# FlagArihant2000/sfm-mvs

Hardware: AMD Instinct MI355X
Metric: descriptor-pair distances/sec (BF-KNN k=2 + Lowe ratio) (higher is better)
Workload: dtype f32 results (bit-identical to the direct-form f32 reference); filter arithmetic on MFMA: i8 MFMA on the descriptors QUANTISED to 8 bits (one grid per pair; the certificate uses the measured residua...; 1 GPU; BASELINE configs[1]: 10k x 10k uniform[0,1) float32 128-D descriptors, BF-KNN k=2 + Lowe ratio 0.70; a step = one launch set = a batch of 8 distinct pairs of that shape per GPU (8e8 distances; 8 distinct pairs per launch set, 2 sets of images rotating over the steps); nq=10000, nt=10000, dim=128

## Files before the change

include/sfm_hip.h:

```cpp
#ifndef SFM_HIP_H
#define SFM_HIP_H

#include <stddef.h>
#include <stdint.h>

#ifdef __cplusplus
extern "C" {
#endif

#define SFM_ABI_VERSION 3

#define SFM_OK             0
#define SFM_ERR_ARG       -1
#define SFM_ERR_WORKSPACE -2
#define SFM_ERR_DEVICE    -3

int         sfm_abi_version(void);
const char* sfm_last_error(void);
const char* sfm_build_id(void);

#define SFM_KNN_FILTER_AUTO      0
#define SFM_KNN_FILTER_F32       1
#define SFM_KNN_FILTER_SPLIT     2
#define SFM_KNN_FILTER_LDS       3
// ... 142 lines not shown
int sfm_host_p3p(const double* K_host, const double* Xw_host, const double* uv_host, double* R_host, double* t_host,
                 int32_t* ok_host);
int sfm_host_five_point(const double* x1n_host, const double* x2n_host, double* E_host, int32_t* count_host);
int sfm_host_decompose_essential(const double* E_host, double* R1_host, double* R2_host, double* t_host);
int sfm_host_pnp_dlt_init(const double* K_host, const double* X_host, const double* uv_host, int64_t n,
                          double* rvec_host, double* tvec_host, int32_t* status_host);
int sfm_host_rodrigues(const double* src_host, int src_is_matrix, double* dst_host, double* jac_host);

int sfm_bgr2gray_u8(const uint8_t* bgr_dev, int64_t w, int64_t h, int64_t stride_bytes, uint8_t* gray_dev, void* stream);
int sfm_pyrdown_u8(const uint8_t* src_dev, int64_t w, int64_t h, int channels, uint8_t* dst_dev, void* stream);
size_t sfm_sift_ws_bytes(int64_t w, int64_t h, int n_octave_layers, int64_t max_keypoints);
int sfm_sift_detect_and_compute(const uint8_t* gray_dev, int64_t w, int64_t h, int64_t stride_bytes,
                                int n_octave_layers, double contrast_threshold, double edge_threshold,
                                double sigma, int64_t max_keypoints, float* keypoints_dev,
                                float* descriptors_dev, int32_t* count_dev, void* ws, size_t ws_bytes,
                                void* stream);

int sfm_mvs_plane_sweep(const uint8_t* ref_dev, const uint8_t* const* src_dev, const float* mv_host, int nsrc, int64_t w, int64_t h,
                        const float* invd_dev, int ndepth, int radius, int topk, float var_min, float cost_max,
                        float* depth_dev, float* cost_dev, int32_t* plane_dev, float* volume_dev, void* stream);
int sfm_mvs_consistency(const float* depth_dev, const float* const* nbr_depth_dev, const int32_t* nbr_index_host,
                        const float* ab_host, int nview, int ref_index, const float* bc_host, int64_t w, int64_t h, float tau,
                        int min_consistent, int unique, uint8_t* mask_dev, float* xyz_dev, void* stream);

int sfm_mvs_cost_shift(const float* volume_dev, int64_t w, int64_t h, int ndepth, int shift, uint16_t* q_dev, void* stream);
int sfm_mvs_cost_aggregate(const uint16_t* q_dev, int64_t w, int64_t h, int ndepth, int p1, int p2, int ndir, uint16_t* s_dev,
                           void* stream);
int sfm_mvs_cost_depth(const uint16_t* s_dev, const uint16_t* q_dev, const float* invd_dev, int64_t w, int64_t h, int ndepth, int gate,
                       float* depth_dev, float* cost_dev, int32_t* plane_dev, void* stream);

int sfm_tsdf_integrate(const float* depth_dev, const uint8_t* mask_dev, const uint8_t* bgr_dev, const float* P_dev, int nview, int64_t w,
                       int64_t h, const float* origin_host, float voxel, int64_t nx, int64_t ny, int64_t nz, float trunc, float* S_dev,
                       float* W_dev, float* CWc_dev, void* stream);
size_t sfm_mesh_count_ws_bytes(int64_t nx, int64_t ny, int64_t nz);
int sfm_mesh_count(const float* S_dev, const float* W_dev, int64_t nx, int64_t ny, int64_t nz, float w_min, int32_t* counts_dev,
                   void* ws_dev, size_t ws_bytes, void* stream);
size_t sfm_mesh_extract_ws_bytes(int64_t nx, int64_t ny, int64_t nz);
int sfm_mesh_extract(const float* S_dev, const float* W_dev, const float* CWc_dev, const float* origin_host, float voxel, int64_t nx,
                     int64_t ny, int64_t nz, float w_min, int64_t max_vertices, int64_t max_faces, float* vertices_dev, float* colors_dev,
                     int32_t* faces_dev, void* ws_dev, size_t ws_bytes, void* stream);

size_t sfm_mesh_components_ws_bytes(int64_t nv, int64_t nf);
int sfm_mesh_components(const int32_t* faces_dev, int64_t nv, int64_t nf, int rounds, int resume, int32_t* labels_dev, int32_t* status_dev,
                        void* ws_dev, size_t ws_bytes, void* stream);
size_t sfm_mesh_clean_ws_bytes(int64_t nv, int64_t nf);
int sfm_mesh_clean(const float* vertices_dev, const float* colors_dev, const int32_t* faces_dev, int64_t nv, int64_t nf,
                   const int32_t* labels_dev, int64_t min_faces, int largest_only, float* out_vertices_dev, float* out_colors_dev,
                   int32_t* out_faces_dev, int32_t* counts_dev, void* ws_dev, size_t ws_bytes, void* stream);

int sfm_profile_enable(int on);
int sfm_debug_set_trace(void* dev_buf);
int sfm_debug_knn_split_delay(int workgroup, int microseconds);
int sfm_debug_knn_prep_general(int on);
int sfm_profile_read(int slot, double* total_ms_host, int64_t* launches_host);
int64_t sfm_host_sync_count(void);
int sfm_pnp_profile_read(double* out10_host, int reset);
int64_t sfm_host_poll_count(void);
int sfm_debug_pnp_sweep_server(int on);

#ifdef __cplusplus
}
#endif
#endif
```

sfm_mvs_amd/_lib.py:

```python
import ctypes
import os

import torch

_HERE = os.path.dirname(os.path.abspath(__file__))
LIB_PATH = os.environ.get("SFM_HIP_LIB") or os.path.join(_HERE, "lib", "libsfmhip.so")

ABI_VERSION = 3


class SfmHipError(RuntimeError):
    """A libsfmhip.so entry point returned a negative status."""


_c = ctypes
_i64, _i32, _int, _f32, _f64, _sz, _vp = (_c.c_int64, _c.c_int32, _c.c_int, _c.c_float, _c.c_double,
                                          _c.c_size_t, _c.c_void_p)

SIGNATURES = {
    "sfm_abi_version": (_int, []),
    "sfm_last_error": (_c.c_char_p, []),
    "sfm_build_id": (_c.c_char_p, []),
    "sfm_knn2_l2_f32_ws_bytes": (_sz, [_i64, _i64, _int, _int]),
    "sfm_knn2_l2_f32": (_int, [_vp, _i64, _i64, _vp, _i64, _i64, _int, _int, _vp, _vp, _vp, _vp, _sz, _vp]),
# ... 23 lines not shown
    "sfm_ba_schur_solve": (_int, [_vp, _i64, _vp, _vp, _i64, _i64, _vp, _vp, _vp, _vp, _f64, _int, _f64, _int, _vp, _vp,
                                  _c.POINTER(_i32), _c.POINTER(_i32), _vp, _sz, _vp]),
    "sfm_ba_schur_indexed_ws_bytes": (_sz, [_i64]),
    "sfm_ba_schur_indexed": (_int, [_vp, _i64, _vp, _vp, _i64, _i64, _vp, _vp, _i64, _int, _vp, _vp, _vp, _sz, _vp]),
    "sfm_block_inverse": (_int, [_vp, _i64, _int, _vp, _vp]),
    "sfm_block_inverse_checked": (_int, [_vp, _i64, _int, _vp, _vp, _vp]),
    "sfm_block_matvec": (_int, [_vp, _vp, _i64, _int, _vp, _vp]),
    "sfm_norm_l2_ws_bytes": (_sz, []),
    "sfm_norm_l2": (_int, [_vp, _vp, _i64, _int, _vp, _vp, _sz, _vp]),
    "sfm_host_epnp": (_int, [_vp, _vp, _vp, _int, _vp, _vp]),
    "sfm_selftest_mfma_accumulation": (_int, [_int, _int, _vp, _vp, _sz, _vp]),
    "sfm_knn_mfma_selftest_result": (_int, [_c.POINTER(_f64), _c.POINTER(_f32)]),
    "sfm_host_p3p": (_int, [_vp, _vp, _vp, _vp, _vp, _vp]),
    "sfm_host_five_point": (_int, [_vp, _vp, _vp, _vp]),
    "sfm_host_decompose_essential": (_int, [_vp, _vp, _vp, _vp]),
    "sfm_host_pnp_dlt_init": (_int, [_vp, _vp, _vp, _i64, _vp, _vp, _vp]),
    "sfm_host_rodrigues": (_int, [_vp, _int, _vp, _vp]),
    "sfm_project_points_f64": (_int, [_vp, _vp, _vp, _vp, _i64, _vp, _vp]),
    "sfm_find_essential_mat_ws_bytes": (_sz, [_i64]),
    "sfm_find_essential_mat": (_int, [_vp, _vp, _i64, _vp, _f64, _f64, _int, _vp, _vp, _vp, _vp, _sz, _vp]),
    "sfm_recover_pose_ws_bytes": (_sz, [_i64]),
    "sfm_recover_pose": (_int, [_vp, _vp, _vp, _i64, _vp, _f64, _int, _vp, _vp, _vp, _vp, _vp, _sz, _vp]),
    "sfm_solve_pnp_ransac_ws_bytes": (_sz, [_i64]),
    "sfm_solve_pnp_ransac": (_int, [_vp, _vp, _i64, _vp, _int, _f32, _f64, _vp, _vp, _vp, _vp, _vp, _sz, _vp]),
    "sfm_bgr2gray_u8": (_int, [_vp, _i64, _i64, _i64, _vp, _vp]),
    "sfm_pyrdown_u8": (_int, [_vp, _i64, _i64, _int, _vp, _vp]),
    "sfm_sift_ws_bytes": (_sz, [_i64, _i64, _int, _i64]),
    "sfm_sift_detect_and_compute": (_int, [_vp, _i64, _i64, _i64, _int, _f64, _f64, _f64, _i64, _vp, _vp, _vp, _vp, _sz, _vp]),
    "sfm_score_essential": (_int, [_vp, _int, _vp, _vp, _i64, _f32, _vp, _vp, _vp]),
    "sfm_recover_pose_score": (_int, [_vp, _int, _vp, _vp, _i64, _f64, _int, _vp, _vp, _vp]),
    "sfm_score_pnp": (_int, [_vp, _int, _vp, _vp, _vp, _i64, _f32, _vp, _vp, _vp]),
    "sfm_mvs_plane_sweep": (_int, [_vp, _vp, _vp, _int, _i64, _i64, _vp, _int, _int, _int, _f32, _f32, _vp, _vp, _vp, _vp, _vp]),
    "sfm_mvs_consistency": (_int, [_vp, _vp, _vp, _vp, _int, _int, _vp, _i64, _i64, _f32, _int, _int, _vp, _vp, _vp]),
    "sfm_mvs_cost_shift": (_int, [_vp, _i64, _i64, _int, _int, _vp, _vp]),
    "sfm_mvs_cost_aggregate": (_int, [_vp, _i64, _i64, _int, _int, _int, _int, _vp, _vp]),
    "sfm_mvs_cost_depth": (_int, [_vp, _vp, _vp, _i64, _i64, _int, _int, _vp, _vp, _vp, _vp]),
    "sfm_tsdf_integrate": (_int, [_vp, _vp, _vp, _vp, _int, _i64, _i64, _vp, _f32, _i64, _i64, _i64, _f32, _vp, _vp, _vp, _vp]),
    "sfm_mesh_count_ws_bytes": (_sz, [_i64, _i64, _i64]),
    "sfm_mesh_count": (_int, [_vp, _vp, _i64, _i64, _i64, _f32, _vp, _vp, _sz, _vp]),
    "sfm_mesh_extract_ws_bytes": (_sz, [_i64, _i64, _i64]),
    "sfm_mesh_extract": (_int, [_vp, _vp, _vp, _vp, _f32, _i64, _i64, _i64, _f32, _i64, _i64, _vp, _vp, _vp, _vp, _sz, _vp]),
    "sfm_mesh_components_ws_bytes": (_sz, [_i64, _i64]),
    "sfm_mesh_components": (_int, [_vp, _i64, _i64, _int, _int, _vp, _vp, _vp, _sz, _vp]),
    "sfm_mesh_clean_ws_bytes": (_sz, [_i64, _i64]),
    "sfm_mesh_clean": (_int, [_vp, _vp, _vp, _i64, _i64, _vp, _i64, _int, _vp, _vp, _vp, _vp, _vp, _sz, _vp]),
    "sfm_profile_enable": (_int, [_int]),
    "sfm_host_sync_count": (_i64, []),
    "sfm_pnp_profile_read": (_int, [_c.POINTER(_f64), _int]),
    "sfm_host_poll_count": (_i64, []),
    "sfm_debug_pnp_sweep_server": (_int, [_int]),
    "sfm_debug_set_trace": (_int, [_vp]),
    "sfm_debug_knn_split_delay": (_int, [_int, _int]),
    "sfm_debug_knn_prep_general": (_int, [_int]),
    "sfm_profile_read": (_int, [_int, _c.POINTER(_f64), _c.POINTER(_i64)]),
}

_lib = None


def lib():
    global _lib
    if _lib is not None:
        return _lib
    if not os.path.exists(LIB_PATH):
        raise ImportError(
            f"{LIB_PATH} is missing: the HIP extension has not been built. "
            "Run `python -c 'import __graft_entry__ as g; g.build()'` (or `make -C sfm_mvs_amd/csrc`). "
            "There is no CPU fallback for the hot path.")
    handle = ctypes.CDLL(LIB_PATH)
    handle.sfm_abi_version.restype = _int
    handle.sfm_abi_version.argtypes = []
    got = handle.sfm_abi_version()
    if got != ABI_VERSION:
        raise ImportError(f"{LIB_PATH}: ABI {got} != binding ABI {ABI_VERSION}; rebuild (python -c 'import __graft_entry__ as g; g.build()')")
    for name, (res, args) in SIGNATURES.items():
        try:
            fn = getattr(handle, name)
        except AttributeError as e:
            raise ImportError(f"{LIB_PATH} (ABI {got}) does not export {name}: header / library mismatch; rebuild") from e
        fn.restype = res
        fn.argtypes = args
    _lib = handle
    return _lib


def build_id():
    return lib().sfm_build_id().decode()


def code_hashes_of_binary():
    return dict(tok.split(":", 1) for tok in build_id().split() if ":" in tok)


def knn_code_hash_of_binary():
    return build_id().split(":", 1)[1].split()[0]


def check(rc, what):
    if rc != 0:
        msg = lib().sfm_last_error()
        raise SfmHipError(f"{what} failed (status {rc}): {msg.decode() if msg else '?'}")


def require_cuda(*tensors):
    for t in tensors:
        if t is not None and not t.is_cuda:
# ... 38 lines not shown
```

sfm_mvs_amd/csrc/knn.hip:

```cpp
#include "common.h"
#include <cfloat>
#include <climits>
#include <cstdlib>
#include <type_traits>
#include <algorithm>
#include <mutex>
#include <vector>

namespace {

typedef float f32x16 __attribute__((ext_vector_type(16)));
typedef float f32x4 __attribute__((ext_vector_type(4)));
typedef float f32x3 __attribute__((ext_vector_type(3), aligned(4)));
typedef int i32x3 __attribute__((ext_vector_type(3), aligned(4)));

constexpr int kDim = 128;
constexpr int kTileT = 32;


constexpr int kResidentWaves = 4096;
constexpr int kMaxSlots = 258;
constexpr float kInf = __builtin_huge_valf();
constexpr int kSubTilesHost = 64;
constexpr int kI8SubTilesHost = 128;
// ... 425 lines not shown
                k1 = m1;
                k0 = lo;
                (void)hi;
            }
            if (!(ABL & 2)) __syncthreads();
        }

        if (qok) {
            flush_keys(k0, k1, k2, sub_t0, h, cand_s + obase + 6 * sub, cand_i + obase + 6 * sub);
            for (int e = sub + 1; e < nsub; ++e)
#pragma unroll
                for (int r = 0; r < 3; ++r) {
                    cand_s[obase + 6 * e + r] = kInf;
                    cand_i[obase + 6 * e + r] = -1;
                }
        }
        u += t_end - t_begin;
    }
    if (trace && threadIdx.x == 0) trace[4 * blockIdx.x + 1] = wall_clock64();
}

typedef __bf16 bf16x8 __attribute__((ext_vector_type(8)));
typedef _Float16 f16x8 __attribute__((ext_vector_type(8)));
typedef unsigned u32x4 __attribute__((ext_vector_type(4)));
typedef _Float16 f16x2 __attribute__((ext_vector_type(2)));
typedef float f32x2 __attribute__((ext_vector_type(2)));

__device__ __forceinline__ float dot8_f16(const uint4& a, const uint4& b, float c) {
    c = __builtin_amdgcn_fdot2(__builtin_bit_cast(f16x2, a.x), __builtin_bit_cast(f16x2, b.x), c, false);
    c = __builtin_amdgcn_fdot2(__builtin_bit_cast(f16x2, a.y), __builtin_bit_cast(f16x2, b.y), c, false);
    c = __builtin_amdgcn_fdot2(__builtin_bit_cast(f16x2, a.z), __builtin_bit_cast(f16x2, b.z), c, false);
    c = __builtin_amdgcn_fdot2(__builtin_bit_cast(f16x2, a.w), __builtin_bit_cast(f16x2, b.w), c, false);
    return c;
}

__device__ __forceinline__ unsigned bf16_rn_bits(float x) {
    const unsigned u = __float_as_uint(x);
    return (u + 0x7FFFu + ((u >> 16) & 1u)) >> 16;
}

constexpr int kModeHalfExact = 0, kModeHalf = 1, kModeSplit = 2;
constexpr int kFlagHalfInexact = 2, kFlagRangeBad = 4, kFlagNotU8 = 8, kFlagSomeU8 = 16;
constexpr int kFlagQ8 = 32;

template <int M>
__device__ __forceinline__ int lane_xor(int v) {
    if constexpr (M == 1) return __builtin_amdgcn_update_dpp(0, v, 0xB1 , 0xF, 0xF, false);
    else if constexpr (M == 2) return __builtin_amdgcn_update_dpp(0, v, 0x4E , 0xF, 0xF, false);
    else if constexpr (M == 4 || M == 8 || M == 16) return __builtin_amdgcn_ds_swizzle(v, 0x1F | (M << 10));
    else return __shfl_xor(v, M, 64);
}
template <int M>
__device__ __forceinline__ float lane_xor(float v) { return __int_as_float(lane_xor<M>(__float_as_int(v))); }
__device__ __forceinline__ int knn_filter_mode(const int* __restrict__ flags, const float* __restrict__ bmax, int lane,
                                               float* tmax_out = nullptr) {
    const int fl = flags[lane] | flags[lane + 64] | flags[lane + 128] | flags[lane + 192];
    float tmax = fmaxf(fmaxf(bmax[lane], bmax[lane + 64]), fmaxf(bmax[lane + 128], bmax[lane + 192]));
#pragma unroll
    for (int m = 32; m >= 1; m >>= 1) tmax = fmaxf(tmax, __shfl_xor(tmax, m, 64));
    if (tmax_out) *tmax_out = tmax;
    if (__any((fl & kFlagRangeBad) != 0)) return kModeSplit;
    if (!__any((fl & kFlagHalfInexact) != 0)) return kModeHalfExact;
    return tmax >= 0.25f ? kModeHalf : kModeSplit;
}

constexpr int kMinfoPairMode = 0, kMinfoBatchMode = kMaxBatch, kMinfoTmax = 16, kMinfoTerr = 24, kMinfoQmax = 32, kMinfoBase = 40, kMinfoI8 = 48,
              kMinfoQ8 = 49,
              kMinfoSub8 = 50,
              kMinfoTicket = 51,
              kMinfoQ8S = 56, kMinfoQ8Lo = 64,
              kMinfoWords = 72;
__device__ __forceinline__ int knn_batch_mode(const int* __restrict__ flags, const float* __restrict__ bmax, int n_pairs, int lane) {
    int mode = kModeHalfExact;
    for (int b = 0; b < n_pairs; ++b) mode = max(mode, knn_filter_mode(flags + b * kNormBlocks, bmax + b * kNormBlocks, lane));
    return mode;
}

constexpr int kFragBytes = 1024;
constexpr int kInitFragBytes = 512;
constexpr int kTileFragBytes = 8 * kFragBytes + kInitFragBytes;

__device__ __forceinline__ uint2 frag_init_operand(float x, bool query_side, int h) {
    unsigned hi = bf16_rn_bits(x), mid = 0, lo = 0;
    if (x < kInf) {
        const float r1 = x - __uint_as_float(hi << 16);
        mid = bf16_rn_bits(r1);
        lo = bf16_rn_bits(r1 - __uint_as_float(mid << 16));
    }
    const unsigned one = 0x3F80u;
    if (query_side) return h == 0 ? make_uint2(one | (one << 16), one | (hi << 16)) : make_uint2(mid | (lo << 16), 0u);
    return h == 0 ? make_uint2(hi | (mid << 16), lo | (one << 16)) : make_uint2(one | (one << 16), 0u);
}

constexpr int kI8Groups = 8;
constexpr int kI8Rows = 4 * kI8Groups * 32;
constexpr int kI8SubTiles = 128;
constexpr int kI8TileBytes = 5 * 1024;
constexpr int kI8QTileBytes = 4 * 1024;
constexpr int kI8CMax = 508031, kI8CMin = -503936;
static_assert(kI8SubTiles == kI8SubTilesHost, "make_plan's copy");
constexpr int kKeyEmptyI = 0x7FFFFF00;

constexpr int kQ8SubTiles = 32;
static_assert(kQ8SubTiles == kQ8SubTilesHost, "make_plan's copy");
struct Q8Grid {
    float lo, s, inv;
    int kind;
};
__device__ __forceinline__ Q8Grid q8_sample_grid(const float* __restrict__ Q, int64_t ldq, int nq, const float* __restrict__ T, int64_t ldt, int nt,
                                                 float* __restrict__ red ) {
    const int sr = threadIdx.x >> 4, c = threadIdx.x & 15;
    const float* qs = Q + (int64_t)(((int64_t)sr * nq) >> 4) * ldq + 8 * c;
    const float* ts = T + (int64_t)(((int64_t)sr * nt) >> 4) * ldt + 8 * c;
    const float4 v0 = *reinterpret_cast<const float4*>(qs), v1 = *reinterpret_cast<const float4*>(qs + 4);
    const float4 v2 = *reinterpret_cast<const float4*>(ts), v3 = *reinterpret_cast<const float4*>(ts + 4);
    const float in[16] = {v0.x, v0.y, v0.z, v0.w, v1.x, v1.y, v1.z, v1.w, v2.x, v2.y, v2.z, v2.w, v3.x, v3.y, v3.z, v3.w};
    float mn = kInf, mx = -kInf, sm = 0.f, sq = 0.f;
    bool bad = false, nonu8 = false;
#pragma unroll
    for (int e = 0; e < 16; ++e) {
        mn = fminf(mn, in[e]);
        mx = fmaxf(mx, in[e]);
        sm += in[e];
        sq = fmaf(in[e], in[e], sq);
        bad = bad || !(fabsf(in[e]) < kInf);
        nonu8 = nonu8 || !(in[e] >= 0.f && in[e] <= 255.f && in[e] == floorf(in[e]));
    }
#pragma unroll
    for (int m = 32; m >= 1; m >>= 1) {
        mn = fminf(mn, __shfl_xor(mn, m, 64));
        mx = fmaxf(mx, __shfl_xor(mx, m, 64));
        sm += __shfl_xor(sm, m, 64);
        sq += __shfl_xor(sq, m, 64);
    }
    const int fl = (__any(bad) ? 1 : 0) | (__any(nonu8) ? 2 : 0);
    __syncthreads();
    if ((threadIdx.x & 63) == 0) {
        red[5 * (threadIdx.x >> 6)] = mn;
        red[5 * (threadIdx.x >> 6) + 1] = mx;
        red[5 * (threadIdx.x >> 6) + 2] = __int_as_float(fl);
        red[5 * (threadIdx.x >> 6) + 3] = sm;
        red[5 * (threadIdx.x >> 6) + 4] = sq;
    }
    __syncthreads();
    int flw = 0;
    mn = red[0]; mx = red[1]; sm = 0.f; sq = 0.f;
#pragma unroll
    for (int w = 0; w < 4; ++w) {
        mn = fminf(mn, red[5 * w]);
        mx = fmaxf(mx, red[5 * w + 1]);
        flw |= __float_as_int(red[5 * w + 2]);
        sm += red[5 * w + 3];
        sq += red[5 * w + 4];
    }
    Q8Grid g{0.f, 1.f, 1.f, 0};
    if (flw & 1) { g.kind = 2; return g; }
    if (!(flw & 2)) return g;
    const float s = (mx - mn) * (1.f / 255.f), mabs = fmaxf(fabsf(mn), fabsf(mx));
    if (!(s >= 1e-12f && s <= 1e30f && s >= 1.52587890625e-05f * mabs)) { g.kind = 2; return g; }
    {
        const float mean = sm * (1.f / 4096.f), var = fmaxf(sq * (1.f / 4096.f) - mean * mean, 0.f);
        if (!((mx - mn) * (mx - mn) <= 25.f * var)) { g.kind = 2; return g; }
    }
    g.lo = mn; g.s = s; g.inv = 1.f / s; g.kind = 1;
    return g;
}

__device__ __forceinline__ float fp16_chunk(const float (&in)[8], float sc, unsigned (&fw)[4], unsigned& flags) {
    fw[0] = fw[1] = fw[2] = fw[3] = 0u;
    float err2 = 0.f;
    unsigned amax = 0u, umin = 0xFFFFFFFFu, dor = 0u;
#pragma unroll
    for (int e = 0; e < 8; ++e) {
        const float ev = sc * in[e];
        const _Float16 hv = (_Float16)ev;
        fw[e >> 1] |= (unsigned)__builtin_bit_cast(unsigned short, hv) << (16 * (e & 1));
        const float dv = ev - (float)hv;
        err2 = fmaf(dv, dv, err2);
        const unsigned ab = __float_as_uint(ev) & 0x7FFFFFFFu;
        amax = max(amax, ab);
        umin = min(umin, ab - 1u);
        dor |= __float_as_uint(dv);
    }
    if (amax > 0x476A6000u ) flags |= kFlagRangeBad;
    const bool has_sub = umin < 0x38800000u - 1u;
    if ((dor & 0x7FFFFFFFu) != 0u || has_sub) flags |= kFlagHalfInexact;
    if (has_sub) {
        err2 = 0.f;
#pragma unroll
        for (int e = 0; e < 8; ++e) {
            const float ev = sc * in[e];
            const float dv = fabsf(ev) < 6.103515625e-5f ? ev : ev - (float)__builtin_bit_cast(_Float16, (unsigned short)(fw[e >> 1] >> (16 * (e & 1))));
            err2 = fmaf(dv, dv, err2);
        }
    }
    return err2;
}

template <typename V>
__device__ __forceinline__ V row16_sum(V v) {
    static_assert(sizeof(V) == 4, "one register");
    auto rot = [](V x, auto ctrl) {
        return __builtin_bit_cast(V, __builtin_amdgcn_update_dpp(0, __builtin_bit_cast(int, x), 0x120 + decltype(ctrl)::value , 0xF, 0xF, true));
    };
    v += rot(v, std::integral_constant<int, 8>{});
    v += rot(v, std::integral_constant<int, 4>{});
    v += rot(v, std::integral_constant<int, 2>{});
// ... 233 lines not shown
            }
            if (!chunk8) flags |= kFlagNotU8;
            else if (real) flags |= kFlagSomeU8;
        }
        float err2 = 0.f;
        const float nrm = (isq || real) ? s : kInf;
        if (!__all(chunk8 && real)) {
        unsigned fw[4];
        err2 = fp16_chunk(in, sc, fw, flags);
        err2 += lane_xor<8>(err2); err2 += lane_xor<4>(err2); err2 += lane_xor<2>(err2); err2 += lane_xor<1>(err2);
        if (!(err2 < kInf)) err2 = 0.f;
        const uint4 packed = make_uint4(fw[0], fw[1], fw[2], fw[3]);
        if (frag) {
            if (!(chunk8 && real))
                *reinterpret_cast<uint4*>((isq ? qfrag : tfrag) + (int64_t)(r >> 5) * kTileFragBytes + (((c >> 1) * 64 + (c & 1) * 32 + (r & 31)) << 4)) = packed;
        } else {
            *reinterpret_cast<uint4*>((isq ? qsplit : tsplit) + (2 * (int64_t)npad + r) * kDim + 8 * c) = packed;
        }
        }
        if (q8pair) {
            err2q += lane_xor<8>(err2q); err2q += lane_xor<4>(err2q); err2q += lane_xor<2>(err2q); err2q += lane_xor<1>(err2q);
            err2 = err2q < kInf ? err2q : kInf;
        }
        if (frag && c < 2 && !isq) *reinterpret_cast<uint2*>(tfrag + (int64_t)(r >> 5) * kTileFragBytes + 8 * kFragBytes + ((c * 32 + (r & 31)) << 3)) = frag_init_operand(nrm, false, c);
        if (c == 0) (isq ? qn : tn)[r] = nrm;
        if (do8) {
            const unsigned long long m8 = __ballot(chunk8 && real);
            if (c == 0) (isq ? rmq : rmt)[r] = (unsigned short)(m8 >> (threadIdx.x & 48));
        }
        if (do8 && __any(chunk8)) {
            const unsigned flip = isq ? 0x7F7F7F7Fu : 0x80808080u;
            const unsigned x0 = real ? lo ^ flip : 0u, x1 = real ? hi ^ flip : 0u;
            int w8 = __builtin_amdgcn_sdot4((int)x0, (int)x0, 8, false);
            w8 = __builtin_amdgcn_sdot4((int)x1, (int)x1, w8, false);
            w8 = __builtin_amdgcn_sdot4((int)x0, 0x02020202, w8, false);
            w8 = __builtin_amdgcn_sdot4((int)x1, 0x02020202, w8, false);
            w8 += lane_xor<8>(w8); w8 += lane_xor<4>(w8); w8 += lane_xor<2>(w8); w8 += lane_xor<1>(w8);
            if (chunk8) {
                unsigned char* img = isq ? qi8 + (int64_t)(r >> 5) * kI8QTileBytes : ti8 + (int64_t)(r >> 5) * kI8TileBytes;
                *reinterpret_cast<uint2*>(img + (c >> 2) * 1024 + ((((c >> 1) & 1) * 32 + (r & 31)) << 4) + ((c & 1) << 3)) = make_uint2(x0, x1);
            }
            if (c == 0) (isq ? wq : wt)[r] = w8;
            if (!isq && real) { w8min = min(w8min, w8); w8max = max(w8max, w8); }
        }
        if (isq) {
            if (c == 0) qerr[r] = err2;
            mxq = fmaxf(mxq, s);
        } else {
            mx = fmaxf(mx, s);
            mxe = fmaxf(mxe, err2);
        }
    }
    }
#pragma unroll
    for (int m = 32; m >= 1; m >>= 1) {
        mx = fmaxf(mx, __shfl_xor(mx, m, 64));
        mxe = fmaxf(mxe, __shfl_xor(mxe, m, 64));
        mxq = fmaxf(mxq, __shfl_xor(mxq, m, 64));
    }
    int wfl = 0;
#pragma unroll
    for (int b = 1; b <= kFlagQ8; b <<= 1) wfl |= __any((flags & b) != 0) ? b : 0;
    __shared__ float wmaxe[kPrepWaves], wmaxq[kPrepWaves];
    __shared__ int w8lo[kPrepWaves], w8hi[kPrepWaves];
    if (do8) {
#pragma unroll
        for (int m = 32; m >= 1; m >>= 1) {
            w8min = min(w8min, __shfl_xor(w8min, m, 64));
            w8max = max(w8max, __shfl_xor(w8max, m, 64));
        }
    }
    if ((threadIdx.x & 63) == 0) {
        wmax[threadIdx.x >> 6] = mx;
        wmaxe[threadIdx.x >> 6] = mxe;
        wmaxq[threadIdx.x >> 6] = mxq;
        wmid[threadIdx.x >> 6] = wfl;
        w8lo[threadIdx.x >> 6] = w8min;
        w8hi[threadIdx.x >> 6] = w8max;
    }
    __syncthreads();
    if (threadIdx.x == 0) {
        float bm = wmax[0], bme = wmaxe[0], bmq = wmaxq[0];
        int fl = wmid[0], lo8 = w8lo[0], hi8 = w8hi[0];
        for (int w = 1; w < kPrepWaves; ++w) {
            bm = fmaxf(bm, wmax[w]);
            bme = fmaxf(bme, wmaxe[w]);
            bmq = fmaxf(bmq, wmaxq[w]);
            fl |= wmid[w];
            lo8 = min(lo8, w8lo[w]);
            hi8 = max(hi8, w8hi[w]);
        }
        bmax[blockIdx.x] = bm;
        bmaxerr[blockIdx.x] = bme;
        bqmax[blockIdx.x] = bmq;
        midflag[blockIdx.x] = fl;
        if (do8) { bwmin[blockIdx.x] = lo8; bwmax[blockIdx.x] = hi8; }
        if (blockIdx.x == 0 && stats) stats[0] = 0;
        if (blockIdx.x == 1 || nblk == 1)
            for (int i = 0; i < nzero; ++i) zero[i] = 0;
    }
}

__device__ __forceinline__ uint4 frag_init_i8(int C, int h) {
    int S = -(C >> 7);
    if (h == 1) S -= max(-15 * 128, min(15 * 127, S));
    unsigned wds[4] = {0u, 0u, 0u, 0u};
#pragma unroll
    for (int k = 0; k < 16; ++k) {
        int d;
        if (h == 0 && k == 0) d = C & 127;
        else { d = max(-128, min(127, S)); S -= d; }
        wds[k >> 2] |= (unsigned)(d & 0xFF) << (8 * (k & 3));
    }
    return make_uint4(wds[0], wds[1], wds[2], wds[3]);
}

constexpr int kSplitThreads = 512;
__global__ __launch_bounds__(kSplitThreads) void knn_split_images_kernel(BatchPtrs P, int B, int64_t ldq, int nq, int nq_pad, int64_t ldt, int nt,
                                                                        int nt_pad, unsigned short* __restrict__ qsplit0,
                                                                        unsigned short* __restrict__ tsplit0, int64_t s_qsplit, int64_t s_tsplit,
                                                                        int* __restrict__ midflag, const float* __restrict__ bmax,
                                                                        int force_mode, unsigned char* __restrict__ qhm0 ,
                                                                        unsigned char* __restrict__ thm0, int64_t s_qhm, int64_t s_thm,
                                                                        float* __restrict__ bmaxerr, const float* __restrict__ bqmax, int* __restrict__ minfo,
                                                                        unsigned char* __restrict__ ti8, int64_t s_ti8, const int* __restrict__ wt, int64_t s_tn,
                                                                        const int* __restrict__ bwmin, const int* __restrict__ bwmax,
                                                                        const unsigned char* __restrict__ qi8, int64_t s_qi8, int64_t s_qn,
                                                                        const unsigned short* __restrict__ rmq, const unsigned short* __restrict__ rmt,
                                                                        unsigned char* __restrict__ qfrag, unsigned char* __restrict__ tfrag, int64_t s_qfrag, int64_t s_tfrag,
                                                                        float* __restrict__ qerr ,
                                                                        int* __restrict__ midflag_r, float* __restrict__ bmaxerr_r ,
                                                                        int delay_wg, long long delay_ticks ) {
    if ((int)blockIdx.x == delay_wg) {
        const long long t0 = wall_clock64();
        while (wall_clock64() - t0 < delay_ticks) __builtin_amdgcn_s_sleep(8);
    }
    __shared__ int smode[kMaxBatch], s8ok[kMaxBatch], s8base[kMaxBatch], s8some[kMaxBatch], sq8[kMaxBatch];
    auto reduce_modes = [&](bool leave ) {
        const int wave = threadIdx.x >> 6, lane = threadIdx.x & 63;
        static_assert(kSplitThreads / 64 >= kMaxBatch, "one wave per pair");
        if (wave < B) {
            float tmax;
            const int m = knn_filter_mode(midflag + wave * kNormBlocks, bmax + wave * kNormBlocks, lane, &tmax);
            const float* be = bmaxerr + wave * kNormBlocks;
            const float* bq = bqmax + wave * kNormBlocks;
            float te = fmaxf(fmaxf(be[lane], be[lane + 64]), fmaxf(be[lane + 128], be[lane + 192]));
            float qm = fmaxf(fmaxf(bq[lane], bq[lane + 64]), fmaxf(bq[lane + 128], bq[lane + 192]));
#pragma unroll
            for (int sh = 32; sh >= 1; sh >>= 1) {
                te = fmaxf(te, __shfl_xor(te, sh, 64));
                qm = fmaxf(qm, __shfl_xor(qm, sh, 64));
            }
// ... 2313 lines not shown
    if (lane == 63) wsum[wave] = incl;
    __syncthreads();
    int woff = 0;
    for (int w = 0; w < wave; ++w) woff += wsum[w];
    int pos = base + woff + incl - mine;
#pragma unroll
    for (int k = 0; k < 4; ++k)
        if (pass & (1u << k)) {
            out_q[pos] = qb + k;
            out_t[pos] = ti[k];
            ++pos;
        }
    if (blockIdx.x == gridDim.x - 1 && threadIdx.x == 255) *out_count = pos;
}

__global__ __launch_bounds__(256) void ratio_scatter_kernel(const int* __restrict__ idx, const float* __restrict__ dist, int nq,
                                                            double ratio, const int* __restrict__ block_count,
                                                            int* __restrict__ out_q, int* __restrict__ out_t,
                                                            int* __restrict__ out_count) {
    ratio_scatter_body(idx, dist, nq, ratio, block_count, out_q, out_t, out_count);
}

__global__ __launch_bounds__(256) void ratio_scatter_batch_kernel(BatchPtrs P, int nq, double ratio, const int* __restrict__ block_count,
                                                                  int count_stride) {
    const int pb = blockIdx.y;
    ratio_scatter_body(P.idx[pb], P.dist[pb], nq, ratio, block_count + pb * count_stride, P.out_q[pb], P.out_t[pb], P.out_count[pb], kRatioSub);
}

__global__ __launch_bounds__(256) void gather_matches_kernel(const float2* __restrict__ kp0, const float2* __restrict__ kp1,
                                                             const int* __restrict__ oq, const int* __restrict__ ot,
                                                             const int* __restrict__ count, int64_t capacity,
                                                             float2* __restrict__ p0, float2* __restrict__ p1) {
    int64_t n = *count;
    if (n > capacity) n = capacity;
    for (int64_t i = blockIdx.x * (int64_t)blockDim.x + threadIdx.x; i < n; i += (int64_t)gridDim.x * blockDim.x) {
        p0[i] = kp0[oq[i]];
        p1[i] = kp1[ot[i]];
    }
}

__global__ void knn_fill_empty_kernel(int* __restrict__ idx, float* __restrict__ dist, int64_t n2, int* __restrict__ stats) {
    const int64_t i = blockIdx.x * (int64_t)blockDim.x + threadIdx.x;
    if (i < n2) {
        idx[i] = -1;
        dist[i] = kInf;
    }
    if (i == 0 && stats) stats[0] = stats[1] = stats[2] = stats[3] = 0;
}

long long* g_trace = nullptr;
int g_split_delay_wg = -1;
long long g_split_delay_ticks = 0;
int g_prep_general = 0;

struct KnnWs {
    unsigned short* qsplit;
    unsigned short* tsplit;
    float* qn;
    float* tn;
    float* bmax;
    float* qerr;
    float* bmaxerr;
    float* bqmax;
    int* midflag;
    int* minfo;
    int64_t* wg_begin;
    int* rb_first;
    int* rb_last;
    int* wg_sbase;
    float* cand_s;
    int* cand_i;
    unsigned char* qfrag;
    unsigned char* tfrag;
    unsigned char* qhm;
    unsigned char* thm;
    int64_t s_qsplit, s_tsplit, s_qn, s_tn, s_cand, s_qfrag, s_tfrag, s_qhm, s_thm;
    unsigned char* qi8;
    unsigned char* ti8;
    int* wq;
    int* wt;
    int* bwmin;
    int* bwmax;
    unsigned short* rmq;
    unsigned short* rmt;
    int* midflag_r;
    float* bmaxerr_r;
    int* keys8;
    int* sttab8;
    int64_t* wg_begin8;
    int* rb_first8;
    int* rb_last8;
    int* wg_sbase8;
    int64_t s_qi8, s_ti8, s_keys8;
    size_t bytes;
};

KnnWs carve_ws(void* ws, int64_t nq, int64_t nt, const Plan& p, const Plan* p8) {
    (void)nt;
    sfm::Carver c(ws);
    KnnWs w{};
    const size_t B = (size_t)p.B;
    w.s_tn = (int64_t)p.tiles * kTileT;
    w.s_qn = p.nq_pad;
    w.s_qsplit = p.q4 ? 0 : (int64_t)p.nq_pad * kDim * 3;
    w.s_tsplit = p.q4 ? 0 : (int64_t)p.tiles * kTileT * kDim * 3;
    w.s_cand = (int64_t)nq * 2 * p.smax * p.nsub * 3;
// ... 163 lines not shown
    if (hipGetDevice(&dev) != hipSuccess || dev < 0 || dev >= 16) {
        sfm::set_error("sfm_knn2_l2_f32: no usable HIP device");
        return -1.f;
    }
    ChainCal& c = g_chain_cal[dev];
    std::call_once(c.once, [&] {
        const char* assume = getenv("SFM_KNN_ASSUME_E");
        double worst = assume && atof(assume) >= 8.0 ? atof(assume) : 0.0;
        {
            void* ws = nullptr;
            hipStream_t st = nullptr;
            if (hipMalloc(&ws, 32768 + 512) != hipSuccess || hipStreamCreateWithFlags(&st, hipStreamNonBlocking) != hipSuccess) {
                if (ws) (void)hipFree(ws);
                return;
            }
            bool ok = true;
            for (int kind = 0; kind < 3 && ok; ++kind) {
                double r[7];
                ok = sfm_selftest_mfma_accumulation(kind, 4, r, ws, 32768 + 512, st) == SFM_OK;
                for (double v : r) worst = std::max(worst, v);
            }
            (void)hipStreamDestroy(st);
            (void)hipFree(ws);
            if (!ok || !(worst < 1e6)) return;
        }
        c.worst = worst;
        c.scale = worst <= 8.0 ? 1.f : (float)(worst / 8.0);
    });
    if (c.scale < 0.f) sfm::set_error("sfm_knn2_l2_f32: the MFMA accumulation self-test could not run on device %d", dev);
    return c.scale;
}

extern "C" int sfm_knn_mfma_selftest_result(double* worst_units, float* chain_scale) {
    const float s = mfma_chain_scale();
    if (s < 0.f) return SFM_ERR_DEVICE;
    int dev = 0;
    (void)hipGetDevice(&dev);
    if (worst_units) *worst_units = g_chain_cal[dev].worst;
    if (chain_scale) *chain_scale = s;
    return SFM_OK;
}

extern "C" int sfm_debug_knn_split_delay(int workgroup, int microseconds) {
    g_split_delay_wg = workgroup;
    g_split_delay_ticks = (long long)(microseconds < 0 ? 0 : microseconds > 100000 ? 100000 : microseconds) * 100;
    return SFM_OK;
}

extern "C" int sfm_debug_knn_prep_general(int on) {
    g_prep_general = on != 0;
    return SFM_OK;
}

extern "C" int sfm_debug_set_trace(void* dev_buf) {
    g_trace = static_cast<long long*>(dev_buf);
    return SFM_OK;
}

namespace {
constexpr int64_t kMaxTrainRows = 4000000;

static_assert(kFilterHalf == 5 && kFilterNoQuant == 6, "include/sfm_hip.h SFM_KNN_FILTER_*");
bool filter_ok(int filter) { return filter >= kFilterAuto && filter <= kFilterNoQuant; }

size_t knn_ws_bytes(int64_t nq, int64_t nt, int dim, int B, int filter) {
    if (nq < 0 || nt < 0 || nt > kMaxTrainRows || dim != kDim || B < 1 || B > kMaxBatch || !filter_ok(filter)) return 0;
    if (B > 1 && filter == kFilterF32) return 0;
    const Plan p = make_plan(nq, nt, B, filter);
    if (!p.i8) return carve_ws(nullptr, nq, nt, p, nullptr).bytes + 256;
    const Plan p8 = make_plan(nq, nt, B, p.q8 ? kFilterI8PlanQ8 : kFilterI8Plan);
    return carve_ws(nullptr, nq, nt, p, &p8).bytes + 256;
}

size_t ratio_ws_bytes(int64_t nq, int B) {
    return sfm::align_up((size_t)B * (size_t)((nq + kRatioBlock - 1) / kRatioBlock * kRatioSub + 1) * sizeof(int), 256) + 256;
}

int knn_batch_impl(int B, const BatchPtrs& P, int64_t nq, int64_t ldq, int64_t nt, int64_t ldt, int dim, int filter, void* ws, size_t ws_bytes,
                   void* stream_, double ratio, int* ratio_counts, int ratio_stride) {
    SFM_CHECK_ARG(dim == kDim, "sfm_knn2_l2_f32: dim must be 128 (got %d)", dim);
    SFM_CHECK_ARG(B >= 1 && B <= kMaxBatch, "sfm_match_batch_l2_f32: 1 <= batch <= %d (got %d)", kMaxBatch, B);
    SFM_CHECK_ARG(filter_ok(filter), "sfm_knn2_l2_f32: filter must be 0 (auto), 1 (fp32 MFMA), 2 (bf16 split pinned), 3 / 4 (LDS-ring kernel, auto / split), 5 (16-bit only), 6 (auto, never quantised) (got %d)", filter);
    SFM_CHECK_ARG(nq >= 0 && nt >= 0 && nq < INT_MAX / 256 && nt <= kMaxTrainRows, "sfm_knn2_l2_f32: bad sizes nq=%lld nt=%lld (nt <= %lld)",
                  (long long)nq, (long long)nt, (long long)kMaxTrainRows);
    if (nq == 0) return SFM_OK;
    for (int b = 0; b < B; ++b) {
        SFM_CHECK_ARG(P.q[b] && P.idx[b] && P.dist[b] && (P.t[b] || nt == 0), "sfm_knn2_l2_f32: null pointer");
        SFM_CHECK_ARG(((uintptr_t)P.q[b] & 15) == 0 && ((uintptr_t)P.t[b] & 15) == 0, "sfm_knn2_l2_f32: q/t must be 16-byte aligned");
        SFM_CHECK_ARG(((uintptr_t)P.idx[b] & 7) == 0 && ((uintptr_t)P.dist[b] & 7) == 0, "sfm_knn2_l2_f32: idx/dist must be 8-byte aligned");
    }
    SFM_CHECK_ARG(ldq >= dim && ldt >= dim && ldq % 4 == 0 && ldt % 4 == 0, "sfm_knn2_l2_f32: ldq/ldt must be >= dim and multiples of 4");
    hipStream_t stream = sfm::as_stream(stream_);
    if (nt == 0) {
        for (int b = 0; b < B; ++b)
            hipLaunchKernelGGL(knn_fill_empty_kernel, dim3((unsigned)((2 * nq + 255) / 256)), dim3(256), 0, stream, P.idx[b], P.dist[b], 2 * nq, P.stats[b]);
        SFM_CHECK_LAUNCH();
        return SFM_OK;
    }
    SFM_CHECK_ARG(B == 1 || filter != kFilterF32, "sfm_match_batch_l2_f32: the fp32-MFMA filter variant is single-pair");
    const Plan p = make_plan(nq, nt, B, filter);
    Plan p8{};
    if (p.i8) p8 = make_plan(nq, nt, B, p.q8 ? kFilterI8PlanQ8 : kFilterI8Plan);
    const size_t need = knn_ws_bytes(nq, nt, dim, B, filter);
    if (!ws || ws_bytes < need) {
        sfm::set_error("sfm_knn2_l2_f32: workspace too small (%zu < %zu)", ws_bytes, need);
        return SFM_ERR_WORKSPACE;
    }
    char* base = reinterpret_cast<char*>(sfm::align_up((size_t)(uintptr_t)ws, 256));
    const KnnWs w = carve_ws(base, nq, nt, p, p.i8 ? &p8 : nullptr);
    const int nstr8 = p.i8 ? p8.smax * p8.nsub : 0;

    const dim3 grid((unsigned)p.G);
    const int prof_reps = p.split ? sfm::prof_repeat() : 1;
    static const int abl = dev_env_int("SFM_KNN_ABL", 0);
    if (p.split) {
        hipLaunchKernelGGL(knn_prep_kernel, dim3(kNormBlocks + 2, (unsigned)B), dim3(kPrepThreads), 0, stream, P, ldq, (int)nq, p.nq_pad, ldt, (int)nt,
                           p.tiles * kTileT, w.qsplit, w.qn, w.tsplit, w.tn, w.bmax, w.midflag, w.qerr, w.bmaxerr, w.bqmax, w.s_qsplit, w.s_tsplit, w.s_qn, w.s_tn,
                           p.q4 ? w.qfrag : nullptr, w.tfrag, w.s_qfrag, w.s_tfrag,
                           ratio_counts, 0 ,
                           p.units, p.tiles, p.G, p.seg_cost, p.n_rb, w.wg_begin, w.rb_first, w.rb_last, p.q4 ? w.wg_sbase : nullptr,
                           w.qi8, w.ti8, w.s_qi8, w.s_ti8, w.wq, w.wt, w.bwmin, w.bwmax, w.rmq, w.rmt, p8.units, p8.G, p8.n_rb, w.wg_begin8, w.rb_first8,
                           w.rb_last8, w.wg_sbase8, p.q8, w.minfo, g_prep_general);
        SFM_CHECK_LAUNCH();
        hipLaunchKernelGGL(knn_split_images_kernel, dim3(kNormBlocks), dim3(kSplitThreads), 0, stream, P, B, ldq, (int)nq, p.nq_pad, ldt, (int)nt,
                           p.tiles * kTileT, w.qsplit, w.tsplit, w.s_qsplit, w.s_tsplit, w.midflag, w.bmax, p.force_mode,
                           p.q4 ? w.qhm : nullptr, w.thm, w.s_qhm, w.s_thm, w.bmaxerr, w.bqmax, w.minfo, w.ti8, w.s_ti8, w.wt, w.s_tn, w.bwmin, w.bwmax,
                           w.qi8, w.s_qi8, w.s_qn, w.rmq, w.rmt, w.qfrag, w.tfrag, w.s_qfrag, w.s_tfrag, w.qerr, w.midflag_r, w.bmaxerr_r, g_split_delay_wg, g_split_delay_ticks);
        SFM_CHECK_LAUNCH();
        sfm::prof_begin(sfm::kProfKnnFilter, stream);
#define SFM_LAUNCH_SPLIT2(A, WV)                                                                                        \
    hipLaunchKernelGGL((knn_filter_split2_kernel<A, WV>), grid, dim3(64 * WV), kRingLdsBytes + (WV == 4 ? kQScratchBytes : 0), stream, w.qsplit, w.qn,    \
                       (int)nq, p.nq_pad, w.tsplit, (int)nt, p.tiles * kTileT, w.tn, p.tiles, p.units, p.smax, p.nsub,    \
                       w.midflag, w.bmax, p.force_mode, w.cand_s, w.cand_i, w.wg_begin, w.rb_first, p.n_rb1, B, w.s_qsplit, w.s_tsplit,    \
                       w.s_qn, w.s_tn, w.s_cand, w.minfo, w.bmaxerr, g_trace)
        for (int rep = 0; rep < prof_reps; ++rep) {
        if (p.q4) {
#define SFM_LAUNCH_Q4(A)                                                                                                                         \
    hipLaunchKernelGGL(knn_filter_q4_kernel<A>, grid, dim3(256), 0, stream, w.qfrag, w.tfrag, w.qhm, w.thm, (int)nq, p.nq_pad, p.tiles, p.smax, p.nsub, \
                       w.midflag, w.bmax, p.force_mode, w.cand_s, w.cand_i, w.wg_begin, w.rb_first, p.n_rb1, B, w.s_qfrag, w.s_tfrag, w.s_qhm,         \
                       w.s_thm, w.s_cand, w.minfo, w.bmaxerr, w.wg_sbase, g_trace, w.qi8, w.ti8, w.s_qi8, w.s_ti8, w.keys8, w.sttab8, w.s_keys8, nstr8,         \
                       w.wg_begin8, p8.n_rb1, w.wg_sbase8, p8.G, (int)nt)
            if (abl == 1) SFM_LAUNCH_Q4(1); else if (abl == 2) SFM_LAUNCH_Q4(2); else if (abl == 3) SFM_LAUNCH_Q4(3); else if (abl == 4) SFM_LAUNCH_Q4(4); else SFM_LAUNCH_Q4(0);
#undef SFM_LAUNCH_Q4
        } else if (p.waves == 4) {
            if (abl == 1) SFM_LAUNCH_SPLIT2(1, 4); else if (abl == 2) SFM_LAUNCH_SPLIT2(2, 4); else if (abl == 4) SFM_LAUNCH_SPLIT2(4, 4);
            else if (abl == 6) SFM_LAUNCH_SPLIT2(6, 4); else if (abl == 7) SFM_LAUNCH_SPLIT2(7, 4); else SFM_LAUNCH_SPLIT2(0, 4);
        } else if (p.waves == 16) {
            if (abl == 1) SFM_LAUNCH_SPLIT2(1, 16); else if (abl == 7) SFM_LAUNCH_SPLIT2(7, 16); else SFM_LAUNCH_SPLIT2(0, 16);
        } else {
            if (abl == 1) SFM_LAUNCH_SPLIT2(1, 8); else if (abl == 7) SFM_LAUNCH_SPLIT2(7, 8); else SFM_LAUNCH_SPLIT2(0, 8);
        }
        }
#undef SFM_LAUNCH_SPLIT2
    } else {
    const float* q = P.q[0];
    const float* t = P.t[0];
    hipLaunchKernelGGL(knn_norms_kernel, dim3(kNormBlocks + 1), dim3(256), 0, stream, t, ldt, (int)nt, w.tn, w.bmax,
                       P.stats[0], ratio_counts, 0, p.units, p.tiles, p.G, p.seg_cost, p.n_rb, w.wg_begin, w.rb_first, w.rb_last);
    SFM_CHECK_LAUNCH();
    sfm::prof_begin(sfm::kProfKnnFilter, stream);
#define SFM_LAUNCH_FILTER(A, WV)                                                                                     \
    hipLaunchKernelGGL((knn_filter_kernel<A, WV>), grid, dim3(64 * WV), kLdsFloats * sizeof(float), stream, q, ldq,    \
                       (int)nq, t, ldt, (int)nt, w.tn, p.tiles, p.units, p.smax, p.nsub, w.cand_s, w.cand_i, g_trace)
    if (p.waves == 4) {
        switch (abl) {
            case 1: SFM_LAUNCH_FILTER(1, 4); break;
            case 7: SFM_LAUNCH_FILTER(7, 4); break;
            default: SFM_LAUNCH_FILTER(0, 4); break;
        }
// ... 166 lines not shown
```

Baseline: 4841 billion distances/s.

## Shrink prep grid to one resident round and use permlane/DPP wave reductions

The prep kernel grid per pair is reduced from kNormBlocks to roughly one resident round of workgroups split across the batch, with a debug override. Blocks beyond the grid get their per-block max/flag slots zeroed by a strided loop. Wave-wide reductions switch from shfl_xor butterflies to permlane32/16 swaps plus DPP row rotates. The per-element inf and u8 checks are replaced by one fraction flag, with range and finiteness derived from the reduced min, max and sum. The smaller grid assumes the prep kernel loops over its rows, which cannot be checked from the visible code.

After: 4910 billion distances/s, median of 6. +1.4%, better.

```diff
diff --git a/include/sfm_hip.h b/include/sfm_hip.h
--- a/include/sfm_hip.h
+++ b/include/sfm_hip.h
@@ -218,6 +218,7 @@
 int sfm_debug_set_trace(void* dev_buf);
 int sfm_debug_knn_split_delay(int workgroup, int microseconds);
 int sfm_debug_knn_prep_general(int on);
+int sfm_debug_knn_prep_blocks(int n);
 int sfm_profile_read(int slot, double* total_ms_host, int64_t* launches_host);
 int64_t sfm_host_sync_count(void);
 int sfm_pnp_profile_read(double* out10_host, int reset);
diff --git a/sfm_mvs_amd/_lib.py b/sfm_mvs_amd/_lib.py
--- a/sfm_mvs_amd/_lib.py
+++ b/sfm_mvs_amd/_lib.py
@@ -99,6 +99,7 @@
     "sfm_debug_set_trace": (_int, [_vp]),
     "sfm_debug_knn_split_delay": (_int, [_int, _int]),
     "sfm_debug_knn_prep_general": (_int, [_int]),
+    "sfm_debug_knn_prep_blocks": (_int, [_int]),
     "sfm_profile_read": (_int, [_int, _c.POINTER(_f64), _c.POINTER(_i64)]),
 }
 
diff --git a/sfm_mvs_amd/csrc/knn.hip b/sfm_mvs_amd/csrc/knn.hip
--- a/sfm_mvs_amd/csrc/knn.hip
+++ b/sfm_mvs_amd/csrc/knn.hip
@@ -501,6 +501,22 @@
 }
 template <int M>
 __device__ __forceinline__ float lane_xor(float v) { return __int_as_float(lane_xor<M>(__float_as_int(v))); }
+template <typename V, typename Op>
+__device__ __forceinline__ V wave64_reduce(V v, Op op) {
+    static_assert(sizeof(V) == 4, "one register");
+    const auto r32 = __builtin_amdgcn_permlane32_swap(__builtin_bit_cast(unsigned, v), __builtin_bit_cast(unsigned, v), false, false);
+    v = op(__builtin_bit_cast(V, (unsigned)r32[0]), __builtin_bit_cast(V, (unsigned)r32[1]));
+    const auto r16 = __builtin_amdgcn_permlane16_swap(__builtin_bit_cast(unsigned, v), __builtin_bit_cast(unsigned, v), false, false);
+    v = op(__builtin_bit_cast(V, (unsigned)r16[0]), __builtin_bit_cast(V, (unsigned)r16[1]));
+    auto rot = [](V x, auto ctrl) {
+        return __builtin_bit_cast(V, __builtin_amdgcn_update_dpp(0, __builtin_bit_cast(int, x), 0x120 + decltype(ctrl)::value , 0xF, 0xF, true));
+    };
+    v = op(v, rot(v, std::integral_constant<int, 8>{}));
+    v = op(v, rot(v, std::integral_constant<int, 4>{}));
+    v = op(v, rot(v, std::integral_constant<int, 2>{}));
+    v = op(v, rot(v, std::integral_constant<int, 1>{}));
+    return v;
+}
 __device__ __forceinline__ int knn_filter_mode(const int* __restrict__ flags, const float* __restrict__ bmax, int lane,
                                                float* tmax_out = nullptr) {
     const int fl = flags[lane] | flags[lane + 64] | flags[lane + 128] | flags[lane + 192];
@@ -565,24 +581,20 @@
     const float4 v2 = *reinterpret_cast<const float4*>(ts), v3 = *reinterpret_cast<const float4*>(ts + 4);
     const float in[16] = {v0.x, v0.y, v0.z, v0.w, v1.x, v1.y, v1.z, v1.w, v2.x, v2.y, v2.z, v2.w, v3.x, v3.y, v3.z, v3.w};
     float mn = kInf, mx = -kInf, sm = 0.f, sq = 0.f;
-    bool bad = false, nonu8 = false;
+    bool frac = false;
 #pragma unroll
     for (int e = 0; e < 16; ++e) {
         mn = fminf(mn, in[e]);
         mx = fmaxf(mx, in[e]);
         sm += in[e];
         sq = fmaf(in[e], in[e], sq);
-        bad = bad || !(fabsf(in[e]) < kInf);
-        nonu8 = nonu8 || !(in[e] >= 0.f && in[e] <= 255.f && in[e] == floorf(in[e]));
-    }
-#pragma unroll
-    for (int m = 32; m >= 1; m >>= 1) {
-        mn = fminf(mn, __shfl_xor(mn, m, 64));
-        mx = fmaxf(mx, __shfl_xor(mx, m, 64));
-        sm += __shfl_xor(sm, m, 64);
-        sq += __shfl_xor(sq, m, 64);
-    }
-    const int fl = (__any(bad) ? 1 : 0) | (__any(nonu8) ? 2 : 0);
+        frac = frac || in[e] != floorf(in[e]);
+    }
+    mn = wave64_reduce(mn, [](float a, float b) { return fminf(a, b); });
+    mx = wave64_reduce(mx, [](float a, float b) { return fmaxf(a, b); });
+    sm = wave64_reduce(sm, [](float a, float b) { return a + b; });
+    sq = wave64_reduce(sq, [](float a, float b) { return a + b; });
+    const int fl = __any(frac) ? 2 : 0;
     __syncthreads();
     if ((threadIdx.x & 63) == 0) {
         red[5 * (threadIdx.x >> 6)] = mn;
@@ -602,6 +614,8 @@
         sm += red[5 * w + 3];
         sq += red[5 * w + 4];
     }
+    if (!(fabsf(sm) < kInf)) flw |= 1;
+    if (!(mn >= 0.f && mx <= 255.f)) flw |= 2;
     Q8Grid g{0.f, 1.f, 1.f, 0};
     if (flw & 1) { g.kind = 2; return g; }
     if (!(flw & 2)) return g;
@@ -941,23 +955,16 @@
         }
     }
     }
-#pragma unroll
-    for (int m = 32; m >= 1; m >>= 1) {
-        mx = fmaxf(mx, __shfl_xor(mx, m, 64));
-        mxe = fmaxf(mxe, __shfl_xor(mxe, m, 64));
-        mxq = fmaxf(mxq, __shfl_xor(mxq, m, 64));
-    }
-    int wfl = 0;
-#pragma unroll
-    for (int b = 1; b <= kFlagQ8; b <<= 1) wfl |= __any((flags & b) != 0) ? b : 0;
+    auto umax = [](unsigned a, unsigned b) { return max(a, b); };
+    mx = __uint_as_float(wave64_reduce(__float_as_uint(mx), umax));
+    mxe = __uint_as_float(wave64_reduce(__float_as_uint(mxe), umax));
+    mxq = __uint_as_float(wave64_reduce(__float_as_uint(mxq), umax));
+    const int wfl = (int)wave64_reduce(flags, [](unsigned a, unsigned b) { return a | b; });
     __shared__ float wmaxe[kPrepWaves], wmaxq[kPrepWaves];
     __shared__ int w8lo[kPrepWaves], w8hi[kPrepWaves];
     if (do8) {
-#pragma unroll
-        for (int m = 32; m >= 1; m >>= 1) {
-            w8min = min(w8min, __shfl_xor(w8min, m, 64));
-            w8max = max(w8max, __shfl_xor(w8max, m, 64));
-        }
+        w8min = wave64_reduce(w8min, [](int a, int b) { return min(a, b); });
+        w8max = wave64_reduce(w8max, [](int a, int b) { return max(a, b); });
     }
     if ((threadIdx.x & 63) == 0) {
         wmax[threadIdx.x >> 6] = mx;
@@ -987,6 +994,13 @@
         if (blockIdx.x == 0 && stats) stats[0] = 0;
         if (blockIdx.x == 1 || nblk == 1)
             for (int i = 0; i < nzero; ++i) zero[i] = 0;
+    }
+    for (int e = blockIdx.x + nblk * (1 + (int)threadIdx.x); e < kNormBlocks; e += nblk * kPrepThreads) {
+        bmax[e] = 0.f;
+        bmaxerr[e] = 0.f;
+        bqmax[e] = 0.f;
+        midflag[e] = 0;
+        if (do8) { bwmin[e] = INT_MAX; bwmax[e] = INT_MIN; }
     }
 }
 
@@ -3406,6 +3420,13 @@
 int g_split_delay_wg = -1;
 long long g_split_delay_ticks = 0;
 int g_prep_general = 0;
+int g_prep_blocks = 0;
+
+int prep_blocks(int B) {
+    if (g_prep_blocks > 0) return g_prep_blocks;
+    constexpr int kRound = kResidentWaves / (kPrepThreads / 64);
+    return std::min(kNormBlocks, (kRound + B - 1) / B);
+}
 
 struct KnnWs {
     unsigned short* qsplit;
@@ -3675,6 +3696,12 @@
     return SFM_OK;
 }
 
+extern "C" int sfm_debug_knn_prep_blocks(int n) {
+    SFM_CHECK_ARG(n >= 0 && n <= kNormBlocks, "sfm_debug_knn_prep_blocks: 0 (the rule) or 1 .. %d workgroups per pair (got %d)", kNormBlocks, n);
+    g_prep_blocks = n;
+    return SFM_OK;
+}
+
 extern "C" int sfm_debug_set_trace(void* dev_buf) {
     g_trace = static_cast<long long*>(dev_buf);
     return SFM_OK;
@@ -3737,7 +3764,7 @@
     const int prof_reps = p.split ? sfm::prof_repeat() : 1;
     static const int abl = dev_env_int("SFM_KNN_ABL", 0);
     if (p.split) {
-        hipLaunchKernelGGL(knn_prep_kernel, dim3(kNormBlocks + 2, (unsigned)B), dim3(kPrepThreads), 0, stream, P, ldq, (int)nq, p.nq_pad, ldt, (int)nt,
+        hipLaunchKernelGGL(knn_prep_kernel, dim3((unsigned)prep_blocks(B) + 2, (unsigned)B), dim3(kPrepThreads), 0, stream, P, ldq, (int)nq, p.nq_pad, ldt, (int)nt,
                            p.tiles * kTileT, w.qsplit, w.qn, w.tsplit, w.tn, w.bmax, w.midflag, w.qerr, w.bmaxerr, w.bqmax, w.s_qsplit, w.s_tsplit, w.s_qn, w.s_tn,
                            p.q4 ? w.qfrag : nullptr, w.tfrag, w.s_qfrag, w.s_tfrag,
                            ratio_counts, 0 ,
```
